# martellab-sri/ModalTune

Hardware: AMD Instinct MI355X
Metric: slides/sec (train step) at 10k patches x 1536-d (higher is better)
Workload: dtype f16; 1 GPU; Prov-GigaPath ModalAdapter train step, 10000 patches x 1536-d, 6 pathways -> 64 gene tokens + 1 task token, 3 task passes, fp16 operands / fp32 accumulate, 1 slide per GPU per step, task passes as two concurrent groups (B = 2 | 1 on two HIP streams), train mode: Dropout(0.25) on the embedded input and both backbone branches, DropPath(0..0.1) per layer and on the Extractor FFN (Philox masks regener; patches=10000, parallelism=dp1, dropout=True

## Files before the change

modaltune_amd/csrc/adapter.hip:

```cpp
#include "common.h"

namespace {

constexpr int TMAX = 128;

template <int HD>
struct AdDim {
  static_assert(HD == 16 || HD == 32 || HD == 64, "adapter head dim");
  static constexpr int NC = HD / 16, NA = (HD + 31) / 32, NG = HD == 16 ? 2 : 4;
  static constexpr int KP = HD + 8;
  static constexpr int TPV = HD == 16 ? TMAX + 8 : TMAX + 4;
  static constexpr int VP = HD == 16 ? 24 : HD == 32 ? 32 : 96;
  static constexpr float SCALE = HD == 16 ? 0.25f : HD == 32 ? 0.17677669529663687f : 0.125f;
};
template <int HD>
MT_DEVINL h16 scaled_h16(float x) {
  float p = x * AdDim<HD>::SCALE;
  if constexpr (HD == 32) asm volatile("" : "+v"(p));
  return (h16)p;
}
#define AD_DIMS                                                                                                          \
  using Dm = AdDim<HD>;                                                                                                  \
  constexpr int AD = HD, NC = Dm::NC, NA = Dm::NA, NG = Dm::NG, KP = Dm::KP, TPV = Dm::TPV;                              \
  constexpr float ASCALE = Dm::SCALE;                                                                                    \
  (void)NC; (void)NA; (void)NG; (void)KP; (void)TPV; (void)ASCALE;                                                       \
  const int AH = HC ? HC : heads, AE = AH * AD

MT_DEVINL void load16(const h16* p, float* out) {
  const h16x8 a = ldg8(p), b = ldg8(p + 8);
#pragma unroll
  for (int i = 0; i < 8; ++i) { out[i] = (float)a[i]; out[8 + i] = (float)b[i]; }
}
MT_DEVINL void store16(h16* p, const float* v) {
  h16x8 a, b;
#pragma unroll
  for (int i = 0; i < 8; ++i) { a[i] = (h16)v[i]; b[i] = (h16)v[8 + i]; }
  stg8(p, a); stg8(p + 8, b);
}

MT_DEVINL h16x8 cat8h(h16x4 lo, h16x4 hi) { return (h16x8){lo[0], lo[1], lo[2], lo[3], hi[0], hi[1], hi[2], hi[3]}; }

template <int HD, int HC>
__global__ __launch_bounds__(256) void inject_attn_fwd_kernel(const h16* __restrict__ q, int rows_per_pass, const float* __restrict__ k,
                                                              const float* __restrict__ v, int T, int heads, h16* __restrict__ a,
                                                              float* __restrict__ lse) {
  AD_DIMS;
  __shared__ __attribute__((aligned(16))) h16 ksh[TMAX * KP];
  __shared__ __attribute__((aligned(16))) h16 vT[AD * TPV];
  const int h = blockIdx.y, b = blockIdx.z, tid = threadIdx.x;
  const int lane = tid & 63, wave = tid >> 6, hh = lane >> 5, l31 = lane & 31;
  for (int i = tid; i < TMAX * AD; i += 256) {
    const int t = i / AD, d = i % AD;
    const bool ok = t < T;
    ksh[t * KP + d] = (h16)(ok ? k[((long)b * T + t) * AE + h * AD + d] : 0.f);
    vT[d * TPV + t] = (h16)(ok ? v[((long)b * T + t) * AE + h * AD + d] : 0.f);
  }
  __syncthreads();
  const int ntb = (T + 31) / 32;
  const int r = blockIdx.x * 128 + wave * 32 + l31;
  const bool valid = r < rows_per_pass;
  const long m = (long)b * rows_per_pass + (valid ? r : 0);
  const h16x8 zero8 = {0, 0, 0, 0, 0, 0, 0, 0};
  const int drow = HD == 16 ? (l31 & 15) : l31;
  h16x8 qf[NC];
#pragma unroll
  for (int c = 0; c < NC; ++c) qf[c] = valid ? ldg8(q + m * AE + h * AD + 16 * c + 8 * hh) : zero8;
  f32x16 sc[TMAX / 32];
  float mx = -1.0e30f;
#pragma unroll
  for (int tb = 0; tb < TMAX / 32; ++tb) {
    if (tb < ntb) {
#pragma unroll
      for (int i = 0; i < 16; ++i) sc[tb][i] = 0.f;
#pragma unroll
      for (int c = 0; c < NC; ++c) {
        const h16x8 kf = *reinterpret_cast<const h16x8*>(&ksh[(tb * 32 + l31) * KP + 16 * c + 8 * hh]);
        sc[tb] = __builtin_amdgcn_mfma_f32_32x32x16_f16(kf, qf[c], sc[tb], 0, 0, 0);
      }
#pragma unroll
      for (int i = 0; i < 16; ++i) {
        if (tb * 32 + (i & 3) + 8 * (i >> 2) + 4 * hh >= T) sc[tb][i] = -1.0e30f;
        mx = fmaxf(mx, sc[tb][i]);
      }
    }
  }
  mx = fmaxf(mx, __shfl_xor(mx, 32, 64));
  const float c = ASCALE * 1.4426950408889634f;
  f32x16 acc[NA];
#pragma unroll
  for (int j = 0; j < NA; ++j)
#pragma unroll
    for (int i = 0; i < 16; ++i) acc[j][i] = 0.f;
  float l = 0.f;
#pragma unroll
  for (int tb = 0; tb < TMAX / 32; ++tb) {
    if (tb < ntb) {
#pragma unroll
      for (int s2 = 0; s2 < 2; ++s2) {
        h16x8 pf;
#pragma unroll
        for (int e = 0; e < 8; ++e) {
          const float pv = __builtin_amdgcn_exp2f((sc[tb][8 * s2 + e] - mx) * c);
          l += pv;
          pf[e] = (h16)pv;
        }
#pragma unroll
        for (int j = 0; j < NA; ++j) {
          const h16* vr = &vT[(32 * j + drow) * TPV + tb * 32 + 16 * s2 + 4 * hh];
          const h16x8 vf = cat8h(*reinterpret_cast<const h16x4*>(vr), *reinterpret_cast<const h16x4*>(vr + 8));
          acc[j] = __builtin_amdgcn_mfma_f32_32x32x16_f16(vf, pf, acc[j], 0, 0, 0);
        }
      }
    }
  }
  l += __shfl_xor(l, 32, 64);
  if (valid) {
    const float inv = 1.0f / l;
    h16* dst = a + m * AE + h * AD;
#pragma unroll
    for (int j = 0; j < NA; ++j)
#pragma unroll
      for (int g = 0; g < NG; ++g)
        *reinterpret_cast<h16x4*>(dst + 32 * j + 8 * g + 4 * hh) =
            (h16x4){(h16)(acc[j][4 * g] * inv), (h16)(acc[j][4 * g + 1] * inv), (h16)(acc[j][4 * g + 2] * inv), (h16)(acc[j][4 * g + 3] * inv)};
    if (lse && hh == 0) lse[m * AH + h] = mx * ASCALE + __logf(l);
  }
}

constexpr int IBR = 128, ITILES = 4, RSTR = IBR + 8;
template <int HD, int HC, bool DET = false>
__global__ __launch_bounds__(256) void inject_attn_bwd_kernel(const h16* __restrict__ q, const h16* __restrict__ a,
                                                              const float* __restrict__ lse, const h16* __restrict__ da,
                                                              int rows_per_pass, const float* __restrict__ k,
                                                              const float* __restrict__ v, int T, int heads, h16* __restrict__ dq,
                                                              float* __restrict__ dk, float* __restrict__ dv) {
  AD_DIMS;
  extern __shared__ __attribute__((aligned(16))) float smem[];
  const int ntb = (T + 31) / 32, TB = ntb * 32;
  h16* ksh = reinterpret_cast<h16*>(smem);
  h16* vsh = ksh + TB * KP;
  h16* kT = vsh + TB * KP;
  h16* psT = kT + AD * TPV;
  h16* dssT = psT + T * RSTR;
  h16* qT = dssT + T * RSTR;
  h16* daT = qT + AD * RSTR;
  const int h = blockIdx.y, b = blockIdx.z, tid = threadIdx.x;
  const int lane = tid & 63, wave = tid >> 6, hh = lane >> 5, l31 = lane & 31;
  for (int i = tid; i < TB * AD; i += 256) {
    const int t = i / AD, d = i % AD;
    const bool ok = t < T;
    const h16 kv_ = (h16)(ok ? k[((long)b * T + t) * AE + h * AD + d] : 0.f);
    ksh[t * KP + d] = kv_;
    kT[d * TPV + t] = kv_;
    vsh[t * KP + d] = (h16)(ok ? v[((long)b * T + t) * AE + h * AD + d] : 0.f);
  }
  const int drow = HD == 16 ? (l31 & 15) : l31;
  f32x16 acc[TMAX / 64][NA];
#pragma unroll
  for (int j = 0; j < TMAX / 64; ++j)
#pragma unroll
    for (int j2 = 0; j2 < NA; ++j2)
#pragma unroll
      for (int i = 0; i < 16; ++i) acc[j][j2][i] = 0.f;
  const h16x8 zero8 = {0, 0, 0, 0, 0, 0, 0, 0};
  const float c = ASCALE * 1.4426950408889634f;
  __syncthreads();
  for (int tile = 0; tile < ITILES; ++tile) {
    const int r0 = (blockIdx.x * ITILES + tile) * IBR;
    if (r0 >= rows_per_pass) break;
    const int rl = wave * 32 + l31;
    const int r = r0 + rl;
    const bool valid = r < rows_per_pass;
    const long m = (long)b * rows_per_pass + (valid ? r : 0);
    h16x8 qf[NC], daf[NC];
#pragma unroll
    for (int c = 0; c < NC; ++c) {
      qf[c] = valid ? ldg8(q + m * AE + h * AD + 16 * c + 8 * hh) : zero8;
      daf[c] = valid ? ldg8(da + m * AE + h * AD + 16 * c + 8 * hh) : zero8;
    }
    const float nl2 = valid ? -lse[m * AH + h] * 1.4426950408889634f : -1.0e30f;
    float delta = 0.f;
#pragma unroll
    for (int c = 0; c < NC; ++c) {
      const h16x8 af = ldg8(a + m * AE + h * AD + 16 * c + 8 * hh);
#pragma unroll
      for (int e = 0; e < 8; ++e) {
        delta = fmaf((float)af[e], (float)daf[c][e], delta);
        qT[(16 * c + 8 * hh + e) * RSTR + rl] = qf[c][e];
        daT[(16 * c + 8 * hh + e) * RSTR + rl] = daf[c][e];
      }
    }
    delta += __shfl_xor(delta, 32, 64);
    f32x16 dqa[NA];
#pragma unroll
    for (int j = 0; j < NA; ++j)
#pragma unroll
      for (int i = 0; i < 16; ++i) dqa[j][i] = 0.f;
#pragma unroll
    for (int tb = 0; tb < TMAX / 32; ++tb) {
      if (tb < ntb) {
        f32x16 sc, dpv;
#pragma unroll
        for (int i = 0; i < 16; ++i) { sc[i] = 0.f; dpv[i] = 0.f; }
#pragma unroll
        for (int c = 0; c < NC; ++c) {
          const h16x8 kf = *reinterpret_cast<const h16x8*>(&ksh[(tb * 32 + l31) * KP + 16 * c + 8 * hh]);
          const h16x8 vf = *reinterpret_cast<const h16x8*>(&vsh[(tb * 32 + l31) * KP + 16 * c + 8 * hh]);
          sc = __builtin_amdgcn_mfma_f32_32x32x16_f16(kf, qf[c], sc, 0, 0, 0);
          dpv = __builtin_amdgcn_mfma_f32_32x32x16_f16(vf, daf[c], dpv, 0, 0, 0);
        }
        h16x8 dsf[2];
#pragma unroll
        for (int i = 0; i < 16; ++i) {
          const int t = tb * 32 + (i & 3) + 8 * (i >> 2) + 4 * hh;
          const float pv = t < T ? __builtin_amdgcn_exp2f(fmaf(sc[i], c, nl2)) : 0.f;
          const float ds = pv * (dpv[i] - delta) * ASCALE;
          dsf[i >> 3][i & 7] = (h16)ds;
          if (t < T) {
            psT[t * RSTR + rl] = (h16)pv;
            dssT[t * RSTR + rl] = (h16)ds;
          }
        }
#pragma unroll
        for (int s2 = 0; s2 < 2; ++s2) {
#pragma unroll
          for (int j = 0; j < NA; ++j) {
            const h16* kr = &kT[(32 * j + drow) * TPV + tb * 32 + 16 * s2 + 4 * hh];
            const h16x8 ktf = cat8h(*reinterpret_cast<const h16x4*>(kr), *reinterpret_cast<const h16x4*>(kr + 8));
            dqa[j] = __builtin_amdgcn_mfma_f32_32x32x16_f16(ktf, dsf[s2], dqa[j], 0, 0, 0);
          }
        }
      }
    }
    if (valid) {
      h16* dst = dq + m * AE + h * AD;
#pragma unroll
      for (int j = 0; j < NA; ++j)
#pragma unroll
        for (int g = 0; g < NG; ++g)
          *reinterpret_cast<h16x4*>(dst + 32 * j + 8 * g + 4 * hh) =
              (h16x4){(h16)dqa[j][4 * g], (h16)dqa[j][4 * g + 1], (h16)dqa[j][4 * g + 2], (h16)dqa[j][4 * g + 3]};
    }
    __syncthreads();
    const h16* Asrc = (wave & 1) ? psT : dssT;
    const h16* Bsrc = (wave & 1) ? daT : qT;
#pragma unroll
    for (int j = 0; j < TMAX / 64; ++j) {
      const int tb = (wave >> 1) + 2 * j;
      if (tb < ntb) {
        const int trow = min(tb * 32 + l31, T - 1);
#pragma unroll
        for (int kk = 0; kk < IBR / 16; ++kk) {
          const h16x8 afr = *reinterpret_cast<const h16x8*>(&Asrc[trow * RSTR + kk * 16 + hh * 8]);
#pragma unroll
          for (int j2 = 0; j2 < NA; ++j2) {
            const h16x8 bfr = *reinterpret_cast<const h16x8*>(&Bsrc[(32 * j2 + drow) * RSTR + kk * 16 + hh * 8]);
            acc[j][j2] = __builtin_amdgcn_mfma_f32_32x32x16_f16(afr, bfr, acc[j][j2], 0, 0, 0);
          }
        }
      }
    }
    __syncthreads();
  }
  float* dst = (wave & 1) ? dv : dk;
  if (HD != 16 || l31 < AD) {
#pragma unroll
    for (int j = 0; j < TMAX / 64; ++j) {
      const int tb = (wave >> 1) + 2 * j;
      if (tb < ntb) {
#pragma unroll
        for (int j2 = 0; j2 < NA; ++j2)
#pragma unroll
          for (int i = 0; i < 16; ++i) {
            const int t = tb * 32 + (i & 3) + 8 * (i >> 2) + 4 * hh;
            if constexpr (DET) {
              if (t < T) dst[(((long)blockIdx.x * gridDim.z + b) * T + t) * AE + h * AD + 32 * j2 + l31] = acc[j][j2][i];
            } else {
              if (t < T) atomicAdd(&dst[((long)b * T + t) * AE + h * AD + 32 * j2 + l31], acc[j][j2][i]);
            }
          }
      }
    }
  }
}

constexpr int EKT = 32, EFT = 256;
MT_DEVINL h16x4 ad_tr4(const h16* p) {
  s16x4 r = __builtin_amdgcn_ds_read_tr16_b64_v4i16(
      (__attribute__((address_space(3))) s16x4*)(__attribute__((address_space(3))) void*)p);
  return __builtin_bit_cast(h16x4, r);
}
template <int HD, int HC>
__global__ __launch_bounds__(EFT) void extract_attn_fwd_kernel(const float* __restrict__ q, const h16* __restrict__ kv, int T, int L, int heads,
                                                               int keys_per_split, float* __restrict__ part_acc, float* __restrict__ part_ml) {
  AD_DIMS;
  constexpr int VP = Dm::VP, MS = AD + 2, NV = 4 * NG;
  h16* vsh;
  float* mrg;
  if constexpr (HD == 16) {
    __shared__ __attribute__((aligned(16))) h16 vsh_s[4 * 32 * VP];
    __shared__ float mrg_s[4 * TMAX * MS];
    vsh = vsh_s; mrg = mrg_s;
  } else {
    extern __shared__ __attribute__((aligned(16))) float smem[];
    vsh = reinterpret_cast<h16*>(smem);
    mrg = smem + 4 * 32 * VP / 2;
  }
  const int MW = (HD == 16 ? TMAX : T) * MS;
  const int sp = blockIdx.x, h = blockIdx.y, b = blockIdx.z, tid = threadIdx.x;
  const int nsplit = gridDim.x;
  const int lane = tid & 63, wave = tid >> 6, hh = lane >> 5, l31 = lane & 31;
  const int li = lane & 15, tq = li >> 2, tp = li & 3;
  const int ntb = (T + 31) / 32;
  h16x8 qf[TMAX / 32][NC];
  f32x16 acc[TMAX / 32][NA];
  float mrun[TMAX / 32], lrun[TMAX / 32];
#pragma unroll
  for (int tb = 0; tb < TMAX / 32; ++tb) {
    const int t = tb * 32 + l31;
#pragma unroll
    for (int c = 0; c < NC; ++c)
#pragma unroll
      for (int e = 0; e < 8; ++e) qf[tb][c][e] = scaled_h16<HD>(t < T ? q[((long)b * T + t) * AE + h * AD + 16 * c + 8 * hh + e] : 0.f);
#pragma unroll
    for (int j = 0; j < NA; ++j)
#pragma unroll
      for (int i = 0; i < 16; ++i) acc[tb][j][i] = 0.f;
    mrun[tb] = -1.0e30f; lrun[tb] = 0.f;
  }
  const h16x8 zero8 = {0, 0, 0, 0, 0, 0, 0, 0};
  const int kbeg = sp * keys_per_split, kend = min(L, kbeg + keys_per_split);
  h16* vw = vsh + wave * 32 * VP;
  const int dcol = HD == 16 ? 0 : 16 * (l31 >> 4);
  for (int k0 = kbeg + wave * EKT; k0 < kend; k0 += 4 * EKT) {
    const int key = k0 + l31;
    const bool valid = key < kend;
    const h16* row = kv + ((long)b * L + (valid ? key : kbeg)) * (2 * AE) + h * AD + 8 * hh;
    h16x8 kf[NC];
#pragma unroll
    for (int c = 0; c < NC; ++c) {
      kf[c] = valid ? ldg8(row + 16 * c) : zero8;
      const h16x8 vf = valid ? ldg8(row + AE + 16 * c) : zero8;
      *reinterpret_cast<h16x8*>(&vw[l31 * VP + 16 * c + 8 * hh]) = vf;
    }
    h16x8 vt[NA][2];
#pragma unroll
    for (int j = 0; j < NA; ++j)
#pragma unroll
      for (int s2 = 0; s2 < 2; ++s2) {
        const h16* vr = &vw[(s2 * 16 + 4 * hh + tq) * VP + 32 * j + dcol + 4 * tp];
        const h16x4 lo = ad_tr4(vr), hi = ad_tr4(vr + 8 * VP);
        vt[j][s2] = (h16x8){lo[0], lo[1], lo[2], lo[3], hi[0], hi[1], hi[2], hi[3]};
      }
#pragma unroll
    for (int tb = 0; tb < TMAX / 32; ++tb) {
      if (tb < ntb) {
        f32x16 sc;
#pragma unroll
        for (int i = 0; i < 16; ++i) sc[i] = 0.f;
#pragma unroll
        for (int c = 0; c < NC; ++c) sc = __builtin_amdgcn_mfma_f32_32x32x16_f16(kf[c], qf[tb][c], sc, 0, 0, 0);
        float mx = -1.0e30f;
#pragma unroll
        for (int i = 0; i < 16; ++i) {
          if (k0 + (i & 3) + 8 * (i >> 2) + 4 * hh >= kend) sc[i] = -1.0e30f;
          mx = fmaxf(mx, sc[i]);
        }
        mx = fmaxf(mx, __shfl_xor(mx, 32, 64));
        const float mn = fmaxf(mrun[tb], mx);
        const float al = __expf(mrun[tb] - mn);
        float ls = 0.f;
        h16x8 pf[2];
#pragma unroll
        for (int i = 0; i < 16; ++i) {
          const float pv = __expf(sc[i] - mn);
          ls += pv;
          pf[i >> 3][i & 7] = (h16)pv;
        }
        ls += __shfl_xor(ls, 32, 64);
        lrun[tb] = lrun[tb] * al + ls;
        mrun[tb] = mn;
#pragma unroll
        for (int j = 0; j < NA; ++j) {
#pragma unroll
          for (int i = 0; i < NV; ++i) acc[tb][j][i] *= al;
          acc[tb][j] = __builtin_amdgcn_mfma_f32_32x32x16_f16(vt[j][0], pf[0], acc[tb][j], 0, 0, 0);
          acc[tb][j] = __builtin_amdgcn_mfma_f32_32x32x16_f16(vt[j][1], pf[1], acc[tb][j], 0, 0, 0);
        }
      }
    }
  }
#pragma unroll
  for (int tb = 0; tb < TMAX / 32; ++tb) {
    const int t = tb * 32 + l31;
    if (tb < ntb && t < T) {
      float* mr = mrg + wave * MW + t * MS;
#pragma unroll
      for (int j = 0; j < NA; ++j)
#pragma unroll
        for (int i = 0; i < NV; ++i) mr[32 * j + (i & 3) + 8 * (i >> 2) + 4 * hh] = acc[tb][j][i];
      if (hh == 0) { mr[AD] = mrun[tb]; mr[AD + 1] = lrun[tb]; }
    }
  }
  __syncthreads();
  if (tid < T) {
    const float* mt = mrg + tid * MS;
    float m2 = -1.0e30f;
    for (int wv = 0; wv < 4; ++wv) m2 = fmaxf(m2, mt[wv * MW + AD]);
    float l2 = 0.f, a2[AD];
#pragma unroll
    for (int d = 0; d < AD; ++d) a2[d] = 0.f;
    for (int wv = 0; wv < 4; ++wv) {
      const float wgt = __expf(mt[wv * MW + AD] - m2);
      l2 = fmaf(wgt, mt[wv * MW + AD + 1], l2);
#pragma unroll
      for (int d = 0; d < AD; ++d) a2[d] = fmaf(wgt, mt[wv * MW + d], a2[d]);
    }
    const long o = (((long)b * AH + h) * nsplit + sp) * T + tid;
#pragma unroll
    for (int d = 0; d < AD; ++d) part_acc[o * AD + d] = a2[d];
    part_ml[o * 2] = m2; part_ml[o * 2 + 1] = l2;
  }
}

template <int HD, int HC>
__global__ void extract_attn_reduce_kernel(const float* __restrict__ part_acc, const float* __restrict__ part_ml, int T, int nsplit, int heads,
                                           float* __restrict__ out, float* __restrict__ lse) {
  AD_DIMS;
  const int bh = blockIdx.x, b = bh / AH, h = bh % AH, t = threadIdx.x;
  if (t >= T) return;
  float mx = -1.0e30f;
  for (int s = 0; s < nsplit; ++s) mx = fmaxf(mx, part_ml[(((long)bh * nsplit + s) * T + t) * 2]);
  float l = 0.f, acc[AD];
#pragma unroll
  for (int d = 0; d < AD; ++d) acc[d] = 0.f;
  for (int s = 0; s < nsplit; ++s) {
    const long o = ((long)bh * nsplit + s) * T + t;
    const float w = __expf(part_ml[o * 2] - mx);
    l += w * part_ml[o * 2 + 1];
#pragma unroll
    for (int d = 0; d < AD; ++d) acc[d] = fmaf(w, part_acc[o * AD + d], acc[d]);
  }
  const float inv = 1.0f / l;
#pragma unroll
  for (int d = 0; d < AD; ++d) out[((long)b * T + t) * AE + h * AD + d] = acc[d] * inv;
  lse[((long)b * T + t) * AH + h] = mx + __logf(l);
}

constexpr int EBK = 128, ETILES = 4;
template <int HD, int HC, bool DET = false>
__global__ __launch_bounds__(256) void extract_attn_bwd_kernel(const float* __restrict__ q, const h16* __restrict__ kv,
                                                               const float* __restrict__ out, const float* __restrict__ lse,
                                                               const float* __restrict__ dout, int T, int L, int heads, float* __restrict__ dq,
                                                               h16* __restrict__ dkv) {
  AD_DIMS;
  extern __shared__ __attribute__((aligned(16))) float smem[];
  const int ntb = (T + 31) / 32, TB = ntb * 32;
  float* nls = smem;
  float* ndl = nls + TMAX;
  h16* qsh = reinterpret_cast<h16*>(ndl + TMAX);
  h16* dosh = qsh + TB * KP;
  h16* qT = dosh + TB * KP;
  h16* doT = qT + AD * TPV;
  h16* dssT = doT + AD * TPV;
  h16* kT = dssT + T * RSTR;
  const int h = blockIdx.y, b = blockIdx.z, tid = threadIdx.x;
  const int lane = tid & 63, wave = tid >> 6, hh = lane >> 5, l31 = lane & 31;
  for (int i = tid; i < TB * AD; i += 256) {
    const int t = i / AD, d = i % AD;
    const bool ok = t < T;
    const h16 qv_ = scaled_h16<HD>(ok ? q[((long)b * T + t) * AE + h * AD + d] : 0.f);
    const h16 dv_ = (h16)(ok ? dout[((long)b * T + t) * AE + h * AD + d] : 0.f);
    qsh[t * KP + d] = qv_; qT[d * TPV + t] = qv_;
    dosh[t * KP + d] = dv_; doT[d * TPV + t] = dv_;
  }
  for (int t = tid; t < TB; t += 256) {
    float d = 0.f, l = 1.0e30f;
    if (t < T) {
      l = lse[((long)b * T + t) * AH + h];
      for (int e = 0; e < AD; ++e) d = fmaf(dout[((long)b * T + t) * AE + h * AD + e], out[((long)b * T + t) * AE + h * AD + e], d);
    }
    nls[t] = -l; ndl[t] = -d;
  }
  const int drow = HD == 16 ? (l31 & 15) : l31;
  f32x16 accq[NA];
#pragma unroll
  for (int j = 0; j < NA; ++j)
#pragma unroll
    for (int i = 0; i < 16; ++i) accq[j][i] = 0.f;
  const h16x8 zero8 = {0, 0, 0, 0, 0, 0, 0, 0};
  __syncthreads();
  for (int tile = 0; tile < ETILES; ++tile) {
    const int k0 = (blockIdx.x * ETILES + tile) * EBK;
    if (k0 >= L) break;
    const int kl = wave * 32 + l31;
    const int key = k0 + kl;
    const bool valid = key < L;
    const h16* kvrow = kv + ((long)b * L + (valid ? key : 0)) * (2 * AE) + h * AD + 8 * hh;
    h16x8 kf[NC], vf[NC];
#pragma unroll
    for (int c = 0; c < NC; ++c) {
      kf[c] = valid ? ldg8(kvrow + 16 * c) : zero8;
      vf[c] = valid ? ldg8(kvrow + AE + 16 * c) : zero8;
#pragma unroll
      for (int e = 0; e < 8; ++e) kT[(16 * c + 8 * hh + e) * RSTR + kl] = kf[c][e];
    }
    f32x16 dka[NA], dva[NA];
#pragma unroll
    for (int j = 0; j < NA; ++j)
#pragma unroll
      for (int i = 0; i < 16; ++i) { dka[j][i] = 0.f; dva[j][i] = 0.f; }
#pragma unroll
    for (int tb = 0; tb < TMAX / 32; ++tb) {
      if (tb < ntb) {
        f32x16 sc, dpv;
#pragma unroll
        for (int g4 = 0; g4 < 4; ++g4) {
          const f32x4 l4 = *reinterpret_cast<const f32x4*>(&nls[tb * 32 + 8 * g4 + 4 * hh]);
          const f32x4 d4 = *reinterpret_cast<const f32x4*>(&ndl[tb * 32 + 8 * g4 + 4 * hh]);
#pragma unroll
          for (int e = 0; e < 4; ++e) { sc[4 * g4 + e] = l4[e]; dpv[4 * g4 + e] = d4[e]; }
        }
#pragma unroll
        for (int c = 0; c < NC; ++c) {
          const h16x8 qa = *reinterpret_cast<const h16x8*>(&qsh[(tb * 32 + l31) * KP + 16 * c + 8 * hh]);
          const h16x8 da = *reinterpret_cast<const h16x8*>(&dosh[(tb * 32 + l31) * KP + 16 * c + 8 * hh]);
          sc = __builtin_amdgcn_mfma_f32_32x32x16_f16(qa, kf[c], sc, 0, 0, 0);
          dpv = __builtin_amdgcn_mfma_f32_32x32x16_f16(da, vf[c], dpv, 0, 0, 0);
        }
        h16x8 pf[2], dsf[2];
#pragma unroll
        for (int i = 0; i < 16; ++i) {
          const int t = tb * 32 + (i & 3) + 8 * (i >> 2) + 4 * hh;
          const float pv = valid ? __expf(sc[i]) : 0.f;
          const float ds = pv * dpv[i];
          pf[i >> 3][i & 7] = (h16)pv;
          dsf[i >> 3][i & 7] = (h16)ds;
          if (t < T) dssT[t * RSTR + kl] = (h16)(ds * ASCALE);
        }
#pragma unroll
        for (int s2 = 0; s2 < 2; ++s2) {
#pragma unroll
          for (int j = 0; j < NA; ++j) {
            const int toff = (32 * j + drow) * TPV + tb * 32 + 16 * s2 + 4 * hh;
            const h16x8 qtf = cat8h(*reinterpret_cast<const h16x4*>(&qT[toff]), *reinterpret_cast<const h16x4*>(&qT[toff + 8]));
            const h16x8 dtf = cat8h(*reinterpret_cast<const h16x4*>(&doT[toff]), *reinterpret_cast<const h16x4*>(&doT[toff + 8]));
            dka[j] = __builtin_amdgcn_mfma_f32_32x32x16_f16(qtf, dsf[s2], dka[j], 0, 0, 0);
            dva[j] = __builtin_amdgcn_mfma_f32_32x32x16_f16(dtf, pf[s2], dva[j], 0, 0, 0);
          }
        }
      }
    }
    if (valid) {
      h16* dst = dkv + ((long)b * L + key) * (2 * AE) + h * AD;
#pragma unroll
      for (int j = 0; j < NA; ++j) {
#pragma unroll
        for (int g = 0; g < NG; ++g)
          *reinterpret_cast<h16x4*>(dst + 32 * j + 8 * g + 4 * hh) =
              (h16x4){(h16)dka[j][4 * g], (h16)dka[j][4 * g + 1], (h16)dka[j][4 * g + 2], (h16)dka[j][4 * g + 3]};
#pragma unroll
        for (int g = 0; g < NG; ++g)
          *reinterpret_cast<h16x4*>(dst + AE + 32 * j + 8 * g + 4 * hh) =
              (h16x4){(h16)dva[j][4 * g], (h16)dva[j][4 * g + 1], (h16)dva[j][4 * g + 2], (h16)dva[j][4 * g + 3]};
      }
    }
    __syncthreads();
    if (wave < ntb) {
      const int trow = min(wave * 32 + l31, T - 1);
#pragma unroll
      for (int kk = 0; kk < EBK / 16; ++kk) {
        const h16x8 af = *reinterpret_cast<const h16x8*>(&dssT[trow * RSTR + kk * 16 + hh * 8]);
#pragma unroll
        for (int j = 0; j < NA; ++j) {
          const h16x8 bf = *reinterpret_cast<const h16x8*>(&kT[(32 * j + drow) * RSTR + kk * 16 + hh * 8]);
          accq[j] = __builtin_amdgcn_mfma_f32_32x32x16_f16(af, bf, accq[j], 0, 0, 0);
        }
      }
    }
    __syncthreads();
  }
  if ((HD != 16 || l31 < AD) && wave < ntb) {
#pragma unroll
    for (int j = 0; j < NA; ++j)
#pragma unroll
      for (int i = 0; i < 16; ++i) {
        const int t = wave * 32 + (i & 3) + 8 * (i >> 2) + 4 * hh;
        if constexpr (DET) {
          if (t < T) dq[(((long)blockIdx.x * gridDim.z + b) * T + t) * AE + h * AD + 32 * j + l31] = accq[j][i];
        } else {
          if (t < T) atomicAdd(&dq[((long)b * T + t) * AE + h * AD + 32 * j + l31], accq[j][i]);
        }
      }
  }
}

MT_DEVINL f32x4 ld4(const float* p) { return *reinterpret_cast<const f32x4*>(p); }
MT_DEVINL int mha_t4(int T) { return (T + 3) & ~3; }
MT_DEVINL int mha_s1(int T) { const int t4 = mha_t4(T); return ((t4 >> 2) & 1) ? t4 : t4 + 4; }
// ... 209 lines not shown
        }
      }
    }
  }
  if (valid) {
    const float inv = 1.0f / (float)AH;
#pragma unroll
    for (int tb = 0; tb < TMAX / 32; ++tb) {
      if (tb < ntb) {
#pragma unroll
        for (int i = 0; i < 16; ++i) {
          const int t = tb * 32 + (i & 3) + 8 * (i >> 2) + 4 * hh;
          if (t < T) w[((long)b * T + t) * L + key] = acc[tb][i] * inv;
        }
      }
    }
  }
}

MT_DEVINL int probs_stride(int T) { return T | 1; }
template <int HD, int HC>
__global__ __launch_bounds__(256) void inject_attn_probs_kernel(const h16* __restrict__ q, int rows_per_pass, const float* __restrict__ k,
                                                                const float* __restrict__ lse, int T, int heads, int hgroup,
                                                                float* __restrict__ w) {
  AD_DIMS;
  extern __shared__ __attribute__((aligned(16))) float smem[];
  const int ntb = (T + 31) / 32, TB = ntb * 32;
  const int G = HC ? HC : hgroup;
  h16* ksh = reinterpret_cast<h16*>(smem);
  const int b = blockIdx.y, tid = threadIdx.x;
  const int lane = tid & 63, wave = tid >> 6, hh = lane >> 5, l31 = lane & 31;
  const int r0 = blockIdx.x * PBR, rl = wave * 32 + l31;
  const bool valid = r0 + rl < rows_per_pass;
  const long m = (long)b * rows_per_pass + (valid ? r0 + rl : 0);
  const h16x8 zero8 = {0, 0, 0, 0, 0, 0, 0, 0};
  f32x16 acc[TMAX / 32];
#pragma unroll
  for (int tb = 0; tb < TMAX / 32; ++tb)
#pragma unroll
    for (int i = 0; i < 16; ++i) acc[tb][i] = 0.f;
  for (int h0 = 0; h0 < AH; h0 += G) {
    const int gh = min(G, AH - h0), GE = gh * AD;
    if (h0) __syncthreads();
    for (int i = tid; i < TB * GE; i += 256) {
      const int t = i / GE, e = i % GE;
      ksh[((e / AD) * TB + t) * KP + e % AD] = (h16)(t < T ? k[((long)b * T + t) * AE + h0 * AD + e] : 0.f);
    }
    __syncthreads();
    for (int h = 0; h < gh; ++h) {
      h16x8 qf[NC];
#pragma unroll
      for (int c = 0; c < NC; ++c) qf[c] = valid ? ldg8(q + m * AE + (h0 + h) * AD + 16 * c + 8 * hh) : zero8;
      const float nl = valid ? -lse[m * AH + h0 + h] : 0.f;
#pragma unroll
      for (int tb = 0; tb < TMAX / 32; ++tb) {
        if (tb < ntb) {
          f32x16 sc;
#pragma unroll
          for (int i = 0; i < 16; ++i) sc[i] = 0.f;
#pragma unroll
          for (int c = 0; c < NC; ++c) {
            const h16x8 kf = *reinterpret_cast<const h16x8*>(&ksh[(h * TB + tb * 32 + l31) * KP + 16 * c + 8 * hh]);
            sc = __builtin_amdgcn_mfma_f32_32x32x16_f16(kf, qf[c], sc, 0, 0, 0);
          }
#pragma unroll
          for (int i = 0; i < 16; ++i) acc[tb][i] += __expf(fmaf(sc[i], ASCALE, nl));
        }
      }
    }
  }
  __syncthreads();
  const int S = probs_stride(T);
  float* osh = smem;
  const float inv = 1.0f / (float)AH;
  if (valid) {
#pragma unroll
    for (int tb = 0; tb < TMAX / 32; ++tb) {
      if (tb < ntb) {
#pragma unroll
        for (int i = 0; i < 16; ++i) {
          const int t = tb * 32 + (i & 3) + 8 * (i >> 2) + 4 * hh;
          if (t < T) osh[rl * S + t] = acc[tb][i] * inv;
        }
      }
    }
  }
  __syncthreads();
  const int n = min(PBR, rows_per_pass - r0) * T;
  float* dst = w + ((long)b * rows_per_pass + r0) * T;
  for (int e = tid; e < n; e += 256) dst[e] = osh[(e / T) * S + e % T];
}

__global__ void token_probs_mean_kernel(const float* __restrict__ probs, int B, int heads, int T, float* __restrict__ out) {
  const long n = (long)T * T;
  const long e = (long)blockIdx.x * blockDim.x + threadIdx.x;
  if (e >= (long)B * n) return;
  const long b = e / n, r = e % n;
  float s = 0.f;
  for (int h = 0; h < heads; ++h) s += probs[(b * heads + h) * n + r];
  out[e] = s / (float)heads;
}

#define AD_DISPATCH(heads, hd, CALL)                        \
  do {                                                      \
    if ((hd) == 16 && (heads) == 12) return CALL(16, 12);   \
    if ((hd) == 16) return CALL(16, 0);                     \
    if ((hd) == 32) return CALL(32, 0);                     \
    if ((hd) == 64) return CALL(64, 0);                     \
    return MT_ERR_UNSUPPORTED;                              \
  } while (0)

constexpr int LDS_MAX = 160 * 1024;

template <int HD, int HC>
int launch_inject_fwd(const h16* q, int rows_per_pass, int B, const float* k, const float* v, int T, int heads, h16* a, float* lse,
                      hipStream_t stream) {
  hipLaunchKernelGGL((inject_attn_fwd_kernel<HD, HC>), dim3(cdiv(rows_per_pass, 128), heads, B), dim3(256), 0, stream, q, rows_per_pass, k,
                     v, T, heads, a, lse);
  MT_CHECK_LAUNCH();
  return MT_OK;
}

template <int HD, int HC, bool DET = false>
int launch_inject_bwd(const h16* q, const h16* a, const float* lse, const h16* da, int rows_per_pass, int B, const float* k, const float* v,
                      int T, int heads, h16* dq, float* dk, float* dv, hipStream_t stream) {
  using Dm = AdDim<HD>;
  const int TBk = cdiv(T, 32) * 32;
  const size_t shm = sizeof(h16) * ((size_t)2 * TBk * Dm::KP + HD * Dm::TPV + (size_t)(2 * T + 2 * HD) * RSTR);
  if (shm > (size_t)LDS_MAX) return MT_ERR_UNSUPPORTED;
  static bool attr_set = false;
  if (!attr_set) {
    (void)hipFuncSetAttribute((const void*)inject_attn_bwd_kernel<HD, HC, DET>, hipFuncAttributeMaxDynamicSharedMemorySize, LDS_MAX);
    attr_set = true;
  }
  hipLaunchKernelGGL((inject_attn_bwd_kernel<HD, HC, DET>), dim3(cdiv(rows_per_pass, IBR * ITILES), heads, B), dim3(256), shm, stream, q, a, lse,
                     da, rows_per_pass, k, v, T, heads, dq, dk, dv);
  MT_CHECK_LAUNCH();
  return MT_OK;
}

template <int HD, int HC>
int launch_extract_fwd(const float* q, const h16* kv, int B, int T, int L, int heads, int kps, float* out, float* lse, float* part_acc,
                       float* part_ml, int nsplit, hipStream_t stream) {
  const size_t shm = HD == 16 ? 0 : sizeof(h16) * 4 * 32 * AdDim<HD>::VP + sizeof(float) * 4 * (size_t)T * (HD + 2);
  if (HD != 16) {
    static bool attr_set = false;
    if (!attr_set) {
      (void)hipFuncSetAttribute((const void*)extract_attn_fwd_kernel<HD, HC>, hipFuncAttributeMaxDynamicSharedMemorySize, LDS_MAX);
      attr_set = true;
    }
  }
  hipLaunchKernelGGL((extract_attn_fwd_kernel<HD, HC>), dim3(nsplit, heads, B), dim3(EFT), shm, stream, q, kv, T, L, heads, kps, part_acc,
                     part_ml);
  hipLaunchKernelGGL((extract_attn_reduce_kernel<HD, HC>), dim3(B * heads), dim3(TMAX), 0, stream, part_acc, part_ml, T, nsplit, heads, out,
                     lse);
  MT_CHECK_LAUNCH();
  return MT_OK;
}

template <int HD, int HC, bool DET = false>
int launch_extract_bwd(const float* q, const h16* kv, const float* out, const float* lse, const float* dout, int B, int T, int L, int heads,
                       float* dq, h16* dkv, hipStream_t stream) {
  using Dm = AdDim<HD>;
  const int TBk = cdiv(T, 32) * 32;
  const size_t shm = sizeof(float) * (2 * TMAX) + sizeof(h16) * ((size_t)2 * TBk * Dm::KP + 2 * HD * Dm::TPV + (size_t)(T + HD) * RSTR);
  static bool attr_set = false;
  if (!attr_set) {
    (void)hipFuncSetAttribute((const void*)extract_attn_bwd_kernel<HD, HC, DET>, hipFuncAttributeMaxDynamicSharedMemorySize, LDS_MAX);
    attr_set = true;
  }
  hipLaunchKernelGGL((extract_attn_bwd_kernel<HD, HC, DET>), dim3(cdiv(L, EBK * ETILES), heads, B), dim3(256), shm, stream, q, kv, out, lse, dout,
                     T, L, heads, dq, dkv);
  MT_CHECK_LAUNCH();
  return MT_OK;
}

inline int probs_group(int heads, size_t per_head) {
  const int g = (int)((size_t)PROBS_LDS / per_head);
  return g < 1 ? 1 : g > heads ? heads : g;
}

template <int HD, int HC>
int launch_extract_probs(const float* q, const h16* kv, const float* lse, int B, int T, int L, int heads, float* w, hipStream_t stream) {
  const int TBk = cdiv(T, 32) * 32;
  const size_t per_head = sizeof(float) * TBk + sizeof(h16) * (size_t)TBk * AdDim<HD>::KP;
  const int G = HC ? HC : probs_group(heads, per_head);
  const size_t shm = per_head * G;
  static bool attr_set = false;
  if (!attr_set) {
    (void)hipFuncSetAttribute((const void*)extract_attn_probs_kernel<HD, HC>, hipFuncAttributeMaxDynamicSharedMemorySize, LDS_MAX);
    attr_set = true;
  }
  hipLaunchKernelGGL((extract_attn_probs_kernel<HD, HC>), dim3(cdiv(L, PBR), B), dim3(256), shm, stream, q, kv, lse, T, L, heads, G, w);
  MT_CHECK_LAUNCH();
  return MT_OK;
}

template <int HD, int HC>
int launch_inject_probs(const h16* q, int rows_per_pass, int B, const float* k, const float* lse, int T, int heads, float* w,
                        hipStream_t stream) {
  const int TBk = cdiv(T, 32) * 32;
  const size_t per_head = sizeof(h16) * (size_t)TBk * AdDim<HD>::KP;
  const int G = HC ? HC : probs_group(heads, per_head);
  const size_t kimg = per_head * G, otile = sizeof(float) * (size_t)PBR * (T | 1);
  const size_t shm = kimg > otile ? kimg : otile;
  static bool attr_set = false;
  if (!attr_set) {
    (void)hipFuncSetAttribute((const void*)inject_attn_probs_kernel<HD, HC>, hipFuncAttributeMaxDynamicSharedMemorySize, LDS_MAX);
    attr_set = true;
  }
  hipLaunchKernelGGL((inject_attn_probs_kernel<HD, HC>), dim3(cdiv(rows_per_pass, PBR), B), dim3(256), shm, stream, q, rows_per_pass, k, lse,
                     T, heads, G, w);
  MT_CHECK_LAUNCH();
  return MT_OK;
}

template <int HD>
int launch_token_fwd(const float* q, const float* k, const float* v, int B, int T, int E, int heads, float* out, float* probs,
                     hipStream_t stream) {
  const int T4 = (T + 3) & ~3, S1 = ((T4 >> 2) & 1) ? T4 : T4 + 4;
  const size_t shm = sizeof(float) * ((size_t)T * HD + (size_t)T4 * HD + (size_t)T * S1);
  static bool attr_set = false;
  if (!attr_set) {
    (void)hipFuncSetAttribute((const void*)token_mha_fwd_kernel<HD>, hipFuncAttributeMaxDynamicSharedMemorySize, LDS_MAX);
    attr_set = true;
  }
  hipLaunchKernelGGL(token_mha_fwd_kernel<HD>, dim3(heads, B), dim3(512), shm, stream, q, k, v, T, E, heads, out, probs);
  MT_CHECK_LAUNCH();
  return MT_OK;
}

template <int HD, int FORM>
void launch_token_bwd_form(size_t shm, const float* q, const float* k, const float* v, const float* probs, const float* dout, int B, int T,
                           int E, int heads, float* dq, float* dk, float* dv, hipStream_t stream) {
  static bool attr_set = false;
  if (!attr_set) {
    (void)hipFuncSetAttribute((const void*)token_mha_bwd_kernel<HD, FORM>, hipFuncAttributeMaxDynamicSharedMemorySize, LDS_MAX);
    attr_set = true;
  }
  hipLaunchKernelGGL((token_mha_bwd_kernel<HD, FORM>), dim3(heads, B), dim3(512), shm, stream, q, k, v, probs, dout, T, E, heads, dq, dk, dv);
}

template <int HD>
int launch_token_bwd(const float* q, const float* k, const float* v, const float* probs, const float* dout, int B, int T, int E, int heads,
                     float* dq, float* dk, float* dv, hipStream_t stream) {
  const size_t op = sizeof(float) * (size_t)T * HD, tt = sizeof(float) * (size_t)T * (T + 1);
  if (4 * op + 2 * tt <= (size_t)LDS_MAX)
    launch_token_bwd_form<HD, 0>(4 * op + 2 * tt, q, k, v, probs, dout, B, T, E, heads, dq, dk, dv, stream);
  else if (4 * op + tt <= (size_t)LDS_MAX)
    launch_token_bwd_form<HD, 1>(4 * op + tt, q, k, v, probs, dout, B, T, E, heads, dq, dk, dv, stream);
  else
    launch_token_bwd_form<HD, 2>(2 * op + tt, q, k, v, probs, dout, B, T, E, heads, dq, dk, dv, stream);
  MT_CHECK_LAUNCH();
  return MT_OK;
}

inline bool ad_heads_ok(int heads, int head_dim) { return heads >= 1 && head_dim >= 1 && heads <= 1024; }

}

extern "C" int mt_inject_attn_fwd_hd(const mt_half* q, int M, int rows_per_pass, const float* k, const float* v, int T, int heads,
                                     int head_dim, mt_half* a, float* lse, mt_stream_t stream) {
  if (!q || !k || !v || !a || M <= 0 || rows_per_pass <= 0 || M % rows_per_pass || T < 1 || T > TMAX || !ad_heads_ok(heads, head_dim))
    return MT_ERR_BAD_ARG;
#define AD_CALL(HD, HC) \
  launch_inject_fwd<HD, HC>((const h16*)q, rows_per_pass, M / rows_per_pass, k, v, T, heads, (h16*)a, lse, (hipStream_t)stream)
  AD_DISPATCH(heads, head_dim, AD_CALL);
#undef AD_CALL
}

extern "C" int mt_inject_attn_fwd(const mt_half* q, int M, int rows_per_pass, const float* k, const float* v, int T,
                                  mt_half* a, float* lse, mt_stream_t stream) {
  return mt_inject_attn_fwd_hd(q, M, rows_per_pass, k, v, T, 12, 16, a, lse, stream);
}

extern "C" int mt_inject_attn_bwd_hd(const mt_half* q, const mt_half* a, const float* lse, const mt_half* da, int M, int rows_per_pass,
                                     const float* k, const float* v, int T, int heads, int head_dim, mt_half* dq, float* dk, float* dv,
                                     mt_stream_t stream) {
  if (!q || !a || !lse || !da || !k || !v || !dq || !dk || !dv || M <= 0 || rows_per_pass <= 0 || M % rows_per_pass || T < 1 ||
      T > TMAX || !ad_heads_ok(heads, head_dim))
    return MT_ERR_BAD_ARG;
#define AD_CALL(HD, HC)                                                                                                              \
  launch_inject_bwd<HD, HC>((const h16*)q, (const h16*)a, lse, (const h16*)da, rows_per_pass, M / rows_per_pass, k, v, T, heads, (h16*)dq, \
                            dk, dv, (hipStream_t)stream)
  AD_DISPATCH(heads, head_dim, AD_CALL);
#undef AD_CALL
}

extern "C" int mt_inject_attn_bwd(const mt_half* q, const mt_half* a, const float* lse, const mt_half* da, int M,
                                  int rows_per_pass, const float* k, const float* v, int T, mt_half* dq, float* dk,
                                  float* dv, mt_stream_t stream) {
  return mt_inject_attn_bwd_hd(q, a, lse, da, M, rows_per_pass, k, v, T, 12, 16, dq, dk, dv, stream);
}

extern "C" long mt_inject_attn_bwd_hd_det_elems(int M, int rows_per_pass, int T, int heads, int head_dim) {
  if (M <= 0 || rows_per_pass <= 0 || M % rows_per_pass || T < 1 || T > TMAX || !ad_heads_ok(heads, head_dim) ||
      (head_dim != 16 && head_dim != 32 && head_dim != 64))
    return MT_ERR_BAD_ARG;
  return 2L * cdiv(rows_per_pass, IBR * ITILES) * (M / rows_per_pass) * T * heads * head_dim;
}

extern "C" int mt_inject_attn_bwd_hd_det(const mt_half* q, const mt_half* a, const float* lse, const mt_half* da, int M, int rows_per_pass,
                                         const float* k, const float* v, int T, int heads, int head_dim, mt_half* dq, float* dk,
                                         float* dv, float* partials, long partials_elems, mt_stream_t stream) {
  if (!q || !a || !lse || !da || !k || !v || !dq || !dk || !dv || !partials) return MT_ERR_BAD_ARG;
  const long need = mt_inject_attn_bwd_hd_det_elems(M, rows_per_pass, T, heads, head_dim);
  if (need < 0 || partials_elems < need) return MT_ERR_BAD_ARG;
  const int slots = cdiv(rows_per_pass, IBR * ITILES), E = heads * head_dim;
// ... 145 lines not shown
```

Baseline: 24.90 slides/s.

## Remap inject-bwd blocks across XCDs and parallelize extract reduce over head dim

The inject attention backward kernel gets an XCD-aware block remapping, so consecutive logical workgroups land on the same XCD. It also gets occupancy hints in launch bounds (2 blocks for head dim 16) and a reduced unroll of the key-block loop for HD=16 to lower register pressure. The extract attention split-reduce kernel changes from one thread per token looping over all head dims to one thread per (token, dim), with batched loads of split partials, giving more parallelism and coalesced access. The added index math and the changed unrolling could cost some instruction efficiency.

```diff
diff --git a/modaltune_amd/csrc/adapter.hip b/modaltune_amd/csrc/adapter.hip
--- a/modaltune_amd/csrc/adapter.hip
+++ b/modaltune_amd/csrc/adapter.hip
@@ -129,11 +129,12 @@
 
 constexpr int IBR = 128, ITILES = 4, RSTR = IBR + 8;
 template <int HD, int HC, bool DET = false>
-__global__ __launch_bounds__(256) void inject_attn_bwd_kernel(const h16* __restrict__ q, const h16* __restrict__ a,
-                                                              const float* __restrict__ lse, const h16* __restrict__ da,
-                                                              int rows_per_pass, const float* __restrict__ k,
-                                                              const float* __restrict__ v, int T, int heads, h16* __restrict__ dq,
-                                                              float* __restrict__ dk, float* __restrict__ dv) {
+__global__ __launch_bounds__(256, HD == 16 ? 2 : 1) void inject_attn_bwd_kernel(const h16* __restrict__ q, const h16* __restrict__ a,
+                                                                                const float* __restrict__ lse, const h16* __restrict__ da,
+                                                                                int rows_per_pass, const float* __restrict__ k,
+                                                                                const float* __restrict__ v, int T, int heads,
+                                                                                h16* __restrict__ dq, float* __restrict__ dk,
+                                                                                float* __restrict__ dv) {
   AD_DIMS;
   extern __shared__ __attribute__((aligned(16))) float smem[];
   const int ntb = (T + 31) / 32, TB = ntb * 32;
@@ -144,8 +145,12 @@
   h16* dssT = psT + T * RSTR;
   h16* qT = dssT + T * RSTR;
   h16* daT = qT + AD * RSTR;
-  const int h = blockIdx.y, b = blockIdx.z, tid = threadIdx.x;
+  const int nrb = gridDim.x, nwg = nrb * gridDim.y * gridDim.z, lin = blockIdx.x + nrb * (blockIdx.y + gridDim.y * blockIdx.z);
+  const int xq = nwg / 8, xr = nwg % 8, xcd = lin % 8;
+  const int wg = (xcd < xr ? xcd * (xq + 1) : xr * (xq + 1) + (xcd - xr) * xq) + lin / 8;
+  const int h = wg % gridDim.y, rb = (wg / gridDim.y) % nrb, b = wg / (gridDim.y * nrb), tid = threadIdx.x;
   const int lane = tid & 63, wave = tid >> 6, hh = lane >> 5, l31 = lane & 31;
+  constexpr int TBU = HD == 16 ? 1 : TMAX / 32;
   for (int i = tid; i < TB * AD; i += 256) {
     const int t = i / AD, d = i % AD;
     const bool ok = t < T;
@@ -166,7 +171,7 @@
   const float c = ASCALE * 1.4426950408889634f;
   __syncthreads();
   for (int tile = 0; tile < ITILES; ++tile) {
-    const int r0 = (blockIdx.x * ITILES + tile) * IBR;
+    const int r0 = (rb * ITILES + tile) * IBR;
     if (r0 >= rows_per_pass) break;
     const int rl = wave * 32 + l31;
     const int r = r0 + rl;
@@ -196,7 +201,7 @@
     for (int j = 0; j < NA; ++j)
 #pragma unroll
       for (int i = 0; i < 16; ++i) dqa[j][i] = 0.f;
-#pragma unroll
+#pragma unroll TBU
     for (int tb = 0; tb < TMAX / 32; ++tb) {
       if (tb < ntb) {
         f32x16 sc, dpv;
@@ -274,7 +279,7 @@
           for (int i = 0; i < 16; ++i) {
             const int t = tb * 32 + (i & 3) + 8 * (i >> 2) + 4 * hh;
             if constexpr (DET) {
-              if (t < T) dst[(((long)blockIdx.x * gridDim.z + b) * T + t) * AE + h * AD + 32 * j2 + l31] = acc[j][j2][i];
+              if (t < T) dst[(((long)rb * gridDim.z + b) * T + t) * AE + h * AD + 32 * j2 + l31] = acc[j][j2][i];
             } else {
               if (t < T) atomicAdd(&dst[((long)b * T + t) * AE + h * AD + 32 * j2 + l31], acc[j][j2][i]);
             }
@@ -423,28 +428,45 @@
   }
 }
 
+constexpr int ERB = 16;
 template <int HD, int HC>
-__global__ void extract_attn_reduce_kernel(const float* __restrict__ part_acc, const float* __restrict__ part_ml, int T, int nsplit, int heads,
-                                           float* __restrict__ out, float* __restrict__ lse) {
+__global__ __launch_bounds__(256) void extract_attn_reduce_kernel(const float* __restrict__ part_acc, const float* __restrict__ part_ml, int T,
+                                                                  int nsplit, int heads, float* __restrict__ out, float* __restrict__ lse) {
   AD_DIMS;
-  const int bh = blockIdx.x, b = bh / AH, h = bh % AH, t = threadIdx.x;
+  constexpr int ERT = 256 / AD;
+  const int bh = blockIdx.x, b = bh / AH, h = bh % AH, d = threadIdx.x % AD, t = blockIdx.y * ERT + threadIdx.x / AD;
   if (t >= T) return;
+  const float2* ml = reinterpret_cast<const float2*>(part_ml) + (long)bh * nsplit * T + t;
+  const float* pa = part_acc + ((long)bh * nsplit * T + t) * AD + d;
   float mx = -1.0e30f;
-  for (int s = 0; s < nsplit; ++s) mx = fmaxf(mx, part_ml[(((long)bh * nsplit + s) * T + t) * 2]);
-  float l = 0.f, acc[AD];
-#pragma unroll
-  for (int d = 0; d < AD; ++d) acc[d] = 0.f;
-  for (int s = 0; s < nsplit; ++s) {
-    const long o = ((long)bh * nsplit + s) * T + t;
-    const float w = __expf(part_ml[o * 2] - mx);
-    l += w * part_ml[o * 2 + 1];
-#pragma unroll
-    for (int d = 0; d < AD; ++d) acc[d] = fmaf(w, part_acc[o * AD + d], acc[d]);
-  }
-  const float inv = 1.0f / l;
-#pragma unroll
-  for (int d = 0; d < AD; ++d) out[((long)b * T + t) * AE + h * AD + d] = acc[d] * inv;
-  lse[((long)b * T + t) * AH + h] = mx + __logf(l);
+  for (int s0 = 0; s0 < nsplit; s0 += ERB) {
+    float m[ERB];
+#pragma unroll
+    for (int i = 0; i < ERB; ++i) m[i] = ml[(long)min(s0 + i, nsplit - 1) * T].x;
+#pragma unroll
+    for (int i = 0; i < ERB; ++i) mx = fmaxf(mx, m[i]);
+  }
+  float l = 0.f, acc = 0.f;
+  for (int s0 = 0; s0 < nsplit; s0 += ERB) {
+    float2 m[ERB];
+    float a[ERB];
+#pragma unroll
+    for (int i = 0; i < ERB; ++i) {
+      const long s = min(s0 + i, nsplit - 1);
+      m[i] = ml[s * T];
+      a[i] = pa[s * T * AD];
+    }
+#pragma unroll
+    for (int i = 0; i < ERB; ++i) {
+      if (s0 + i < nsplit) {
+        const float w = __expf(m[i].x - mx);
+        l += w * m[i].y;
+        acc = fmaf(w, a[i], acc);
+      }
+    }
+  }
+  out[((long)b * T + t) * AE + h * AD + d] = acc * (1.0f / l);
+  if (d == 0) lse[((long)b * T + t) * AH + h] = mx + __logf(l);
 }
 
 constexpr int EBK = 128, ETILES = 4;
@@ -960,8 +982,8 @@
   }
   hipLaunchKernelGGL((extract_attn_fwd_kernel<HD, HC>), dim3(nsplit, heads, B), dim3(EFT), shm, stream, q, kv, T, L, heads, kps, part_acc,
                      part_ml);
-  hipLaunchKernelGGL((extract_attn_reduce_kernel<HD, HC>), dim3(B * heads), dim3(TMAX), 0, stream, part_acc, part_ml, T, nsplit, heads, out,
-                     lse);
+  hipLaunchKernelGGL((extract_attn_reduce_kernel<HD, HC>), dim3(B * heads, cdiv(T, 256 / HD)), dim3(256), 0, stream, part_acc, part_ml, T,
+                     nsplit, heads, out, lse);
   MT_CHECK_LAUNCH();
   return MT_OK;
 }
```

Measured after the change: 24.92 slides/s, median of 4. About the same (+0.1%).
